# ethz-asl/laser_slam

Hardware: NVIDIA H100
Metric: ICP registrations/s (131072-pt scan vs 524288-pt map, 30 iterations) (higher is better)
Workload: dtype f32

## Files before the change

laser_slam_b200/csrc/ls_grid.cuh:

```cuda
#pragma once
#include <cfloat>
#include <climits>
#include <cstring>

#include <vector_types.h>
#include <vector_functions.h>

#include "ls_math.cuh"

#define LS_FB 8
#define LS_FB3 (LS_FB * LS_FB * LS_FB)
#define LS_PYR_LEVELS 7

namespace ls {

struct Entry {
  uint32_t start;
  int32_t meta;
};

struct Grid {
  float org[3];
  float H0, H1;
  float inv0, inv1;
// ... 113 lines not shown
}
LS_HD float cell_lo(float o, int c, float H) { return o + (float)c * H; }

LS_HD float gap(float q, float lo, float hi, float m) {
  const float a = (lo - m) - q;
  const float b = q - (hi + m);
  return fmaxf(0.0f, fmaxf(a, b));
}

#define LS_SHRINK 0.999999f

LS_HD float ball_radius(float best_d2, float margin) { return sqrtf(best_d2) * 1.000001f + margin; }

LS_HD void Best::offer_pt(float d, const float4& c, int p) { offer(d, f2i(c.w), p); }
LS_HD void TopK::offer_pt(float dist, const float4& c, int p) { offer(dist, f2i(c.w), p); }
template <class Acc>
LS_HD void consider_pt(const float4 p, int pos, float qx, float qy, float qz, Acc& b) {
  b.offer_pt(dist2(qx, qy, qz, p.x, p.y, p.z), p, pos);
}
template <class Acc>
LS_HD void consider(const float4* pts, int pos, float qx, float qy, float qz, Acc& b) {
  consider_pt(ld_pt(pts + pos), pos, qx, qy, qz, b);
}

template <class Acc>
LS_HD void scan_range(const float4* pts, uint32_t a, uint32_t e, float qx, float qy, float qz, Acc& b) {
  uint32_t pos = a;
  for (; pos + 4 <= e; pos += 4) {
    LS_CNT_STEP();
    const float4 p0 = ld_pt(pts + pos), p1 = ld_pt(pts + pos + 1), p2 = ld_pt(pts + pos + 2), p3 = ld_pt(pts + pos + 3);
    consider_pt(p0, (int)pos, qx, qy, qz, b);
    consider_pt(p1, (int)pos + 1, qx, qy, qz, b);
    consider_pt(p2, (int)pos + 2, qx, qy, qz, b);
    consider_pt(p3, (int)pos + 3, qx, qy, qz, b);
  }
  if (pos < e) LS_CNT_STEP();
  for (; pos < e; ++pos) consider(pts, (int)pos, qx, qy, qz, b);
}

template <class Acc>
LS_HD void visit_fine(const Grid& g, const Entry* tab, unsigned long long rows, float lox, float loy, float loz,
                      const float4* pts, float qx, float qy, float qz, Acc& b) {
  const float R = ball_radius(b.bound(), g.margin);
  const int x0 = coord_sub(qx - R, lox, g.inv1), x1 = coord_sub(qx + R, lox, g.inv1);
  const int y0 = coord_sub(qy - R, loy, g.inv1), y1 = coord_sub(qy + R, loy, g.inv1);
  const int z0 = coord_sub(qz - R, loz, g.inv1), z1 = coord_sub(qz + R, loz, g.inv1);
  for (int z = z0; z <= z1; ++z) {
    const float gz = gap(qz, cell_lo(loz, z, g.H1), cell_lo(loz, z + 1, g.H1), g.margin);
    const float gz2 = gz * gz;
    if (gz2 * LS_SHRINK > b.bound()) continue;
    const Entry* row = tab + (z * LS_FB + y0) * LS_FB;
    for (int y = y0; y <= y1; ++y, row += LS_FB) {
      if (!((rows >> (z * LS_FB + y)) & 1ull)) continue;
      const float gy = gap(qy, cell_lo(loy, y, g.H1), cell_lo(loy, y + 1, g.H1), g.margin);
      const float lb = gy * gy + gz2;
      if (lb * LS_SHRINK > b.bound()) continue;
      LS_CNT_STEP();
      const Entry e0 = ld_entry(row + x0);
      const Entry e1 = ld_entry(row + x1);
      scan_range(pts, e0.start, e1.start + (uint32_t)e1.meta, qx, qy, qz, b);
    }
  }
}

template <class Acc>
LS_HD void visit_top_entry(const Grid& g, const GridView& v, const Entry e, unsigned long long rows, float cx, float cy,
                           float cz, float qx, float qy, float qz, Acc& b) {
  if (e.meta > 0) {
    scan_range(v.pts, e.start, e.start + (uint32_t)e.meta, qx, qy, qz, b);
  } else if (e.meta < 0) {
    visit_fine(g, v.tab1 + (size_t)(~e.meta) * LS_FB3, rows, cx, cy, cz, v.pts, qx, qy, qz, b);
  }
}
template <class Acc>
LS_HD void visit_top_cell(const Grid& g, const GridView& v, int x, int y, int z, float cx, float cy, float cz, float qx,
                          float qy, float qz, Acc& b) {
  LS_CNT_STEP();
  const size_t ci = ((size_t)z * g.dim[1] + y) * g.dim[0] + x;
  const Entry e = ld_entry(v.top + ci);
  const unsigned long long rows = ld_rows(v.topmask + ci);
  visit_top_entry(g, v, e, rows, cx, cy, cz, qx, qy, qz, b);
}

template <class Acc>
LS_HDN void pyramid_query(const Grid& g, const GridView& v, float qx, float qy, float qz, Acc& b) {
  int lvl[LS_PYR_LEVELS + 1], bx[LS_PYR_LEVELS + 1], by[LS_PYR_LEVELS + 1], bz[LS_PYR_LEVELS + 1];
  unsigned long long mk[LS_PYR_LEVELS + 1];
  const int* td = g.pdim[g.n_pyr];
  const int n_top = td[0] * td[1] * td[2];
  for (int t = 0; t < n_top; ++t) {
    int sp = 0;
    lvl[0] = g.n_pyr;
    bx[0] = (t % td[0]) * 4;
    by[0] = ((t / td[0]) % td[1]) * 4;
    bz[0] = (t / (td[0] * td[1])) * 4;
    mk[0] = ld_mask(v.pyr + g.poff[g.n_pyr] + t);
    while (sp >= 0) {
      if (mk[sp] == 0ull) { --sp; continue; }
      const int bit = ctz64(mk[sp]);
      mk[sp] &= mk[sp] - 1ull;
      LS_CNT_STEP();
      const int cl = lvl[sp] - 1;
      const int cx = bx[sp] + (bit & 3), cy = by[sp] + ((bit >> 2) & 3), cz = bz[sp] + (bit >> 4);
      const float Hc = g.H0 * (float)(1 << (2 * cl));
      const float lx = cell_lo(g.org[0], cx, Hc), ly = cell_lo(g.org[1], cy, Hc), lz = cell_lo(g.org[2], cz, Hc);
      const float gx = gap(qx, lx, cell_lo(g.org[0], cx + 1, Hc), g.margin);
      const float gy = gap(qy, ly, cell_lo(g.org[1], cy + 1, Hc), g.margin);
      const float gz = gap(qz, lz, cell_lo(g.org[2], cz + 1, Hc), g.margin);
      const float lb = gx * gx + (gy * gy + gz * gz);
      if (lb * LS_SHRINK > b.bound()) continue;
      if (cl == 0) {
        visit_top_cell(g, v, cx, cy, cz, lx, ly, lz, qx, qy, qz, b);
      } else {
        ++sp;
        lvl[sp] = cl;
        bx[sp] = cx * 4; by[sp] = cy * 4; bz[sp] = cz * 4;
        mk[sp] = ld_mask(v.pyr + g.poff[cl] + ((size_t)cz * g.pdim[cl][1] + cy) * g.pdim[cl][0] + cx);
      }
    }
  }
}

template <class Acc>
LS_HD void ball_query(const Grid& g, const GridView& v, float qx, float qy, float qz, Acc& b) {
  const float R = ball_radius(b.bound(), g.margin);
  const int x0 = coord_top(qx - R, g.org[0], g.inv0, g.dim[0]), x1 = coord_top(qx + R, g.org[0], g.inv0, g.dim[0]);
  const int y0 = coord_top(qy - R, g.org[1], g.inv0, g.dim[1]), y1 = coord_top(qy + R, g.org[1], g.inv0, g.dim[1]);
  const int z0 = coord_top(qz - R, g.org[2], g.inv0, g.dim[2]), z1 = coord_top(qz + R, g.org[2], g.inv0, g.dim[2]);
  if ((x1 - x0 + 1) * (y1 - y0 + 1) * (z1 - z0 + 1) > 27 && g.n_pyr > 0) {
    pyramid_query(g, v, qx, qy, qz, b);
    return;
  }
  for (int z = z0; z <= z1; ++z) {
    const float cz = cell_lo(g.org[2], z, g.H0);
    const float gz = gap(qz, cz, cell_lo(g.org[2], z + 1, g.H0), g.margin);
    const float gz2 = gz * gz;
    if (gz2 * LS_SHRINK > b.bound()) continue;
    for (int y = y0; y <= y1; ++y) {
      const float cy = cell_lo(g.org[1], y, g.H0);
      const float gy = gap(qy, cy, cell_lo(g.org[1], y + 1, g.H0), g.margin);
      const float lbyz = gy * gy + gz2;
      if (lbyz * LS_SHRINK > b.bound()) continue;
      for (int x = x0; x <= x1; ++x) {
        const float cx = cell_lo(g.org[0], x, g.H0);
        const float gx = gap(qx, cx, cell_lo(g.org[0], x + 1, g.H0), g.margin);
        const float lb = gx * gx + lbyz;
        if (lb * LS_SHRINK > b.bound()) continue;
        visit_top_cell(g, v, x, y, z, cx, cy, cz, qx, qy, qz, b);
      }
    }
  }
}

LS_HDN void seed_query(const Grid& g, const GridView& v, float qx, float qy, float qz, Best& b) {
  const int cx = coord_top(qx, g.org[0], g.inv0, g.dim[0]);
  const int cy = coord_top(qy, g.org[1], g.inv0, g.dim[1]);
  const int cz = coord_top(qz, g.org[2], g.inv0, g.dim[2]);
  const Entry e = ld_entry(v.top + ((size_t)cz * g.dim[1] + cy) * g.dim[0] + cx);
  if (e.meta == 0) {
    int X = 0, Y = 0, Z = 0;
    const int* td = g.pdim[g.n_pyr];
    const int n_top = td[0] * td[1] * td[2];
    if (n_top > 1) {
      const float Ht = g.H0 * (float)(1 << (2 * g.n_pyr));
      float best_lb = INFINITY;
      for (int t = 0; t < n_top; ++t) {
        if (ld_mask(v.pyr + g.poff[g.n_pyr] + t) == 0ull) continue;
        const int tx = t % td[0], ty = (t / td[0]) % td[1], tz = t / (td[0] * td[1]);
        const float gx = gap(qx, cell_lo(g.org[0], tx, Ht), cell_lo(g.org[0], tx + 1, Ht), 0.f);
        const float gy = gap(qy, cell_lo(g.org[1], ty, Ht), cell_lo(g.org[1], ty + 1, Ht), 0.f);
        const float gz = gap(qz, cell_lo(g.org[2], tz, Ht), cell_lo(g.org[2], tz + 1, Ht), 0.f);
        const float lb = gx * gx + (gy * gy + gz * gz);
        if (lb < best_lb) { best_lb = lb; X = tx; Y = ty; Z = tz; }
      }
    }
    for (int l = g.n_pyr; l >= 1; --l) {
      unsigned long long mask = ld_mask(v.pyr + g.poff[l] + ((size_t)Z * g.pdim[l][1] + Y) * g.pdim[l][0] + X);
      const float Hc = g.H0 * (float)(1 << (2 * (l - 1)));
      float best_lb = INFINITY;
      int best_bit = -1;
      while (mask) {
        const int bit = ctz64(mask);
        mask &= mask - 1ull;
        const int ccx = X * 4 + (bit & 3), ccy = Y * 4 + ((bit >> 2) & 3), ccz = Z * 4 + (bit >> 4);
        const float gx = gap(qx, cell_lo(g.org[0], ccx, Hc), cell_lo(g.org[0], ccx + 1, Hc), 0.f);
        const float gy = gap(qy, cell_lo(g.org[1], ccy, Hc), cell_lo(g.org[1], ccy + 1, Hc), 0.f);
        const float gz = gap(qz, cell_lo(g.org[2], ccz, Hc), cell_lo(g.org[2], ccz + 1, Hc), 0.f);
        const float lb = gx * gx + (gy * gy + gz * gz);
        if (lb < best_lb) { best_lb = lb; best_bit = bit; }
      }
      if (best_bit < 0) return;
      X = X * 4 + (best_bit & 3);
      Y = Y * 4 + ((best_bit >> 2) & 3);
      Z = Z * 4 + (best_bit >> 4);
    }
    const Entry s0 = ld_entry(v.top + ((size_t)Z * g.dim[1] + Y) * g.dim[0] + X);
    if (s0.meta != 0) consider(v.pts, (int)s0.start, qx, qy, qz, b);
    return;
  }
  if (e.meta > 0) { scan_range(v.pts, e.start, e.start + (uint32_t)e.meta, qx, qy, qz, b); return; }
  const float lox = cell_lo(g.org[0], cx, g.H0), loy = cell_lo(g.org[1], cy, g.H0), loz = cell_lo(g.org[2], cz, g.H0);
  const int fx = coord_sub(qx, lox, g.inv1), fy = coord_sub(qy, loy, g.inv1), fz = coord_sub(qz, loz, g.inv1);
  const Entry* tab = v.tab1 + (size_t)(~e.meta) * LS_FB3;
  const Entry e1 = ld_entry(tab + (fz * LS_FB + fy) * LS_FB + fx);
  if (e1.meta != 0) { scan_range(v.pts, e1.start, e1.start + (uint32_t)e1.meta, qx, qy, qz, b); return; }
  const int xa = fx > 0 ? fx - 1 : 0, xb = fx < LS_FB - 1 ? fx + 1 : LS_FB - 1;
  for (int z = (fz > 0 ? fz - 1 : 0); z <= (fz < LS_FB - 1 ? fz + 1 : LS_FB - 1); ++z)
    for (int y = (fy > 0 ? fy - 1 : 0); y <= (fy < LS_FB - 1 ? fy + 1 : LS_FB - 1); ++y) {
      const Entry r0 = ld_entry(tab + (z * LS_FB + y) * LS_FB + xa);
      const Entry r1 = ld_entry(tab + (z * LS_FB + y) * LS_FB + xb);
      scan_range(v.pts, r0.start, r1.start + (uint32_t)r1.meta, qx, qy, qz, b);
    }
  if (b.pos < 0) consider(v.pts, (int)e.start, qx, qy, qz, b);
}

LS_HD Best nn_search(const Grid& g, const GridView& v, float qx, float qy, float qz, int warm_pos, float cap_d2) {
  Best b;
  b.d2 = cap_d2;
  b.idx = INT_MAX;
  b.pos = -1;
  if (g.m <= 0) { b.idx = -1; b.d2 = INFINITY; return b; }
  if (warm_pos >= 0) consider(v.pts, warm_pos, qx, qy, qz, b);
  else seed_query(g, v, qx, qy, qz, b);
  ball_query(g, v, qx, qy, qz, b);
  if (b.pos < 0) { b.idx = -1; b.d2 = INFINITY; }
  return b;
}

#ifndef LS_VK
#define LS_VK 8
#endif
static_assert(LS_VK <= 15, "the list header keeps the candidate count in 4 bits");
#ifndef LS_VL_ABS
#define LS_VL_ABS 0.0f
#endif
#ifndef LS_VL_REL
#define LS_VL_REL 0.5f
#endif
#ifndef LS_VL_SKIN
#define LS_VL_SKIN 4.0f
#endif
#ifndef LS_VL_GATE
#define LS_VL_GATE 1.0f
#endif
struct VLists {
  float4* vq;
  float4* vpts;
  int n;
};

struct Collector {
  float r2;
  int cnt;
  float4* out;
  int stride;
  LS_HD float bound() const { return r2; }
  LS_HD void offer_pt(float d, const float4& c, int p) {
    if (d <= r2) {
      if (cnt < LS_VK) st_state4(out + (size_t)cnt * stride, make_float4(c.x, c.y, c.z, i2f(p)));
      else r2 = -1.0f;
      ++cnt;
    }
  }
};

LS_HD bool vlist_query(const VLists& L, const float4* pts, int i, const float4 v, const float4 c0, float qx, float qy,
                       float qz, float cap_d2, Best& b, float4& cbest) {
  const unsigned int bits = (unsigned int)f2i(v.w);
  if (bits == 0u) return false;
  const int cnt = (int)(bits & 15u);
  const float Rv = i2f((int)(bits & ~15u));
  const float Rc = Rv * 0.999996f - sqrtf(dist2(qx, qy, qz, v.x, v.y, v.z)) * 1.000004f;
  if (!(Rc > 0.0f)) return false;
  b.d2 = cap_d2;
  b.idx = INT_MAX;
  b.pos = -1;
  auto take = [&](const float4 c) {
    const float d = dist2(qx, qy, qz, c.x, c.y, c.z);
    const int cpos = f2i(c.w);
    if (d < b.d2) {
      b.d2 = d;
      b.pos = cpos;
      cbest = c;
    } else if (d == b.d2) {
      if (b.pos < 0 || f2i(ld_pt(pts + cpos).w) < f2i(ld_pt(pts + b.pos).w)) {
        b.pos = cpos;
        cbest = c;
      }
    }
  };
  if (cnt > 0) take(c0);
  for (int k0 = 1; k0 < cnt; k0 += 4) {
    float4 cs[4];
#pragma unroll
    for (int u = 0; u < 4; ++u)
      cs[u] = k0 + u < cnt ? ld_state4(L.vpts + (size_t)(k0 + u) * L.n + i) : make_float4(0.f, 0.f, 0.f, 0.f);
#pragma unroll
    for (int u = 0; u < 4; ++u)
      if (k0 + u < cnt) take(cs[u]);
  }
  return b.d2 * 1.00001f <= Rc * Rc;
}

LS_HD void vlist_build(const Grid& g, const GridView& v, const VLists& L, int i, float qx, float qy, float qz, bool found,
                       float found_d2, float cap_d2, float motion) {
  float Rv;
  if (found) {
    const float want = sqrtf(found_d2);
    const float margin = fmaxf(want * LS_VL_REL, LS_VL_ABS) + 1e-4f;
    if (!(motion * LS_VL_GATE <= margin)) return;
    Rv = want + fminf(margin, fmaxf(0.002f, LS_VL_SKIN * motion));
  } else {
    const float want = sqrtf(cap_d2);
    if (!(motion <= want * 0.125f)) return;
    Rv = want * 1.05f + fminf(want * 0.25f, fmaxf(0.002f, 4.0f * motion));
  }
  if (!(Rv < 3.0e38f)) return;
  Collector c;
  c.r2 = Rv * Rv;
  c.cnt = 0;
  c.out = L.vpts + i;
  c.stride = L.n;
  ball_query(g, v, qx, qy, qz, c);
  float4 head = make_float4(qx, qy, qz, 0.0f);
  if (c.cnt <= LS_VK) head.w = i2f((int)((((unsigned int)f2i(Rv * 0.9999999f)) & ~15u) | (unsigned int)c.cnt));
  st_state4(L.vq + i, head);
}

LS_HDN void knn_search(const Grid& g, const GridView& v, float qx, float qy, float qz, int k, TopK& t) {
  t.reset(k);
  if (g.m <= 0) return;
  const float extent = g.H0 * (float)(g.dim[0] + g.dim[1] + g.dim[2]) + 1.0f;
  float R = g.H1;
  for (int round = 0; round < 64; ++round) {
    t.cap = R * R;
    ball_query(g, v, qx, qy, qz, t);
    if (t.d[k - 1] <= t.cap) break;
    if (R > extent + fabsf(qx - g.org[0]) + fabsf(qy - g.org[1]) + fabsf(qz - g.org[2])) break;
    R = R * 2.0f;
  }
}

LS_HD int top_index(const Grid& g, float x, float y, float z) {
  const int cx = coord_top(x, g.org[0], g.inv0, g.dim[0]);
  const int cy = coord_top(y, g.org[1], g.inv0, g.dim[1]);
  const int cz = coord_top(z, g.org[2], g.inv0, g.dim[2]);
  return (cz * g.dim[1] + cy) * g.dim[0] + cx;
}
LS_HD void top_origin(const Grid& g, int c0, float& lox, float& loy, float& loz) {
  const int cx = c0 % g.dim[0];
  const int cy = (c0 / g.dim[0]) % g.dim[1];
  const int cz = c0 / (g.dim[0] * g.dim[1]);
  lox = cell_lo(g.org[0], cx, g.H0);
  loy = cell_lo(g.org[1], cy, g.H0);
  loz = cell_lo(g.org[2], cz, g.H0);
}
LS_HD int sub_index(float x, float y, float z, float lox, float loy, float loz, float inv) {
  return (coord_sub(z, loz, inv) * LS_FB + coord_sub(y, loy, inv)) * LS_FB + coord_sub(x, lox, inv);
}

LS_HDN void grid_setup(Grid& g, const float* lo, const float* hi, float cell_size, int max_cells, int leaf_split,
                       int m) {
  float H = cell_size > 0.f ? cell_size : 2.0f;
  float ext[3], emax = 0.f, oabs = 0.f;
  for (int a = 0; a < 3; ++a) {
    ext[a] = hi[a] - lo[a];
    if (!(ext[a] >= 0.f)) ext[a] = 0.f;
    emax = fmaxf(emax, ext[a]);
    oabs = fmaxf(oabs, fmaxf(fabsf(lo[a]), fabsf(hi[a])));
  }
  for (int it = 0; it < 40; ++it) {
    const float inv = 1.0f / H;
    double cells = 1.0;
    for (int a = 0; a < 3; ++a) cells *= (double)floorf(ext[a] * inv) + 1.0;
    if (cells <= (double)max_cells) break;
    H = H * 2.0f;
  }
  g.H0 = H;
  g.H1 = H / (float)LS_FB;
  g.inv0 = 1.0f / g.H0;
  g.inv1 = 1.0f / g.H1;
  int n = 1;
  for (int a = 0; a < 3; ++a) {
    g.org[a] = lo[a];
    int d = (int)floorf(ext[a] * g.inv0) + 1;
    if (d < 1) d = 1;
    g.dim[a] = d;
    n *= d;
  }
  g.n_cells0 = n;
  g.margin = (oabs + emax + H) * 1.9073486328125e-06f;
  g.m = m;
  g.leaf_split = leaf_split > 0 ? leaf_split : 32;
  g.n_tab1 = 0;
  g.overflow = 0;
  for (int a = 0; a < 3; ++a) g.pdim[0][a] = g.dim[a];
  g.poff[0] = 0;
  int off = 0, l = 0;
  do {
    ++l;
    for (int a = 0; a < 3; ++a) g.pdim[l][a] = (g.pdim[l - 1][a] + 3) / 4;
    g.poff[l] = off;
    off += g.pdim[l][0] * g.pdim[l][1] * g.pdim[l][2];
  } while ((g.pdim[l][0] > 1 || g.pdim[l][1] > 1 || g.pdim[l][2] > 1) && l < LS_PYR_LEVELS);
  g.n_pyr = l;
  g.n_pyr_cells = off;
}

}
```

laser_slam_b200/csrc/ls_kernels.cuh:

```cuda
#pragma once
#include <cuda_runtime.h>
#include <cooperative_groups.h>

#include "ls_grid.cuh"

namespace ls {

constexpr int kMaxParts = 16;
constexpr int kScanTile = 4096;
constexpr int kScanThreads = 512;
constexpr int kIcpThreads = 512;
constexpr int kIcpCtasPerSm = 1024 / kIcpThreads;
constexpr int kMaxSmooth = 15;
constexpr uint32_t kTag1 = 1u << 31, kKeyMask = (1u << 31) - 1u;
constexpr int kSubShift = 22;
constexpr uint32_t kCellMask = (1u << kSubShift) - 1u;

struct Parts {
  int n_parts;
  int offset[kMaxParts + 1];
  const float4* pts[kMaxParts];
  const float4* nrm[kMaxParts];
  float T[kMaxParts][16];
  int identity[kMaxParts];
// ... 772 lines not shown
__global__ void __launch_bounds__(128) knn_normals_kernel(const BuildState* __restrict__ bs, GridView view,
                                                           const float4* __restrict__ pts ,
                                                           int n, int k, float4* __restrict__ out) {
  __shared__ Grid g;
  if (threadIdx.x == 0) g = bs->grid;
  __syncthreads();
  auto centred = [&](int j) {
    float4 p = __ldg(pts + j);
    p.x = p.x - g.mu[0];
    p.y = p.y - g.mu[1];
    p.z = p.z - g.mu[2];
    return p;
  };
  for (int i = blockIdx.x * blockDim.x + threadIdx.x; i < n; i += gridDim.x * blockDim.x) {
    const float4 q = centred(i);
    TopK t;
    knn_search(g, view, q.x, q.y, q.z, k, t);
    int cnt = 0;
    double mx = 0.0, my = 0.0, mz = 0.0;
    for (int j = 0; j < k; ++j) {
      if (t.id[j] == INT_MAX) break;
      const float4 p = centred(t.id[j]);
      mx = mx + (double)p.x;
      my = my + (double)p.y;
      mz = mz + (double)p.z;
      ++cnt;
    }
    float4 nn = make_float4(0.f, 0.f, 0.f, 0.f);
    if (cnt >= 3) {
      const double inv = 1.0 / (double)cnt;
      mx = mx * inv; my = my * inv; mz = mz * inv;
      double C[9] = {0, 0, 0, 0, 0, 0, 0, 0, 0};
      for (int j = 0; j < cnt; ++j) {
        const float4 p = centred(t.id[j]);
        const double dx = (double)p.x - mx, dy = (double)p.y - my, dz = (double)p.z - mz;
        C[0] = C[0] + dx * dx; C[1] = C[1] + dx * dy; C[2] = C[2] + dx * dz;
        C[4] = C[4] + dy * dy; C[5] = C[5] + dy * dz; C[8] = C[8] + dz * dz;
      }
      C[3] = C[1]; C[6] = C[2]; C[7] = C[5];
      double nv[3];
      smallest_eigvec3(C, nv);
      const double ox = (double)q.x + (double)g.mu[0], oy = (double)q.y + (double)g.mu[1], oz = (double)q.z + (double)g.mu[2];
      const double dot = nv[0] * ox + (nv[1] * oy + nv[2] * oz);
      const double sgn = dot > 0.0 ? -1.0 : 1.0;
      nn = make_float4((float)(sgn * nv[0]), (float)(sgn * nv[1]), (float)(sgn * nv[2]), 0.f);
    }
    out[i] = nn;
  }
}

__device__ __forceinline__ unsigned long long globaltimer_ns() {
  unsigned long long t;
  asm volatile("mov.u64 %0, %%globaltimer;" : "=l"(t));
  return t;
}
#define LS_STAMP(slot)                                                                   \
  do {                                                                                   \
    if (P.phase_ns && cta == 0 && tid == 0) P.phase_ns[iter * 6 + (slot)] = globaltimer_ns(); \
  } while (0)

__device__ __forceinline__ unsigned int ld_relaxed_u32(const unsigned int* p) {
  unsigned int v;
  asm volatile("ld.relaxed.gpu.global.u32 %0, [%1];" : "=r"(v) : "l"(p) : "memory");
  return v;
}
__device__ __forceinline__ void red_release_inc(unsigned int* p) {
  asm volatile("red.release.gpu.global.add.u32 [%0], 1;" ::"l"(p) : "memory");
}
__device__ __forceinline__ unsigned int ld_relaxed_sys_u32(const unsigned int* p) {
  unsigned int v;
  asm volatile("ld.relaxed.sys.global.u32 %0, [%1];" : "=r"(v) : "l"(p) : "memory");
  return v;
}
__device__ __forceinline__ unsigned long long ld_relaxed_sys_u64(const unsigned long long* p) {
  unsigned long long v;
  asm volatile("ld.relaxed.sys.global.u64 %0, [%1];" : "=l"(v) : "l"(p) : "memory");
  return v;
}
__device__ __forceinline__ void red_release_sys_inc(unsigned int* p) {
  asm volatile("red.release.sys.global.add.u32 [%0], 1;" ::"l"(p) : "memory");
}

__device__ __forceinline__ void problem_barrier(unsigned int* ctr, unsigned int n_ctas, unsigned int& epoch) {
  __syncthreads();
  if (threadIdx.x == 0) {
    epoch += n_ctas;
    red_release_inc(ctr);
    unsigned int polls = 0;
    unsigned long long t0 = 0ull;
    while (ld_relaxed_u32(ctr) < epoch) {
      __nanosleep(64);
      if ((++polls & 0x3fffu) == 0u) {
        const unsigned long long now = globaltimer_ns();
        if (t0 == 0ull) t0 = now;
        else if (now - t0 > 8000000000ull) {
          printf("[ls] icp_kernel barrier timeout: block %d waits for %u, counter %u\n", (int)blockIdx.x, epoch, ld_relaxed_u32(ctr));
          __trap();
        }
      }
    }
  }
  __syncthreads();
}

struct SelectOut {
  unsigned int bin, rem, total;
};
constexpr size_t kWorkWords = sizeof(IcpWork) / 4;
static_assert(sizeof(IcpWork) % 16 == 0 && offsetof(IcpWork, hist) % 16 == 0 && offsetof(IcpWork, acc) % 16 == 0, "sections move as uint4");

__device__ __forceinline__ void shard_exchange(const IcpProblem& P, IcpWork* X, int cta, unsigned int G, unsigned int& epoch,
                                               unsigned int& xepoch, int off0, int n0, int off1, int n1, int off2, int n2) {
  problem_barrier(&X->barrier, G, epoch);
  const int peers = P.shard_count - 1;
  if (cta < peers) {
    const int g = cta + (cta >= P.shard_rank ? 1 : 0);
    const uint4* src = reinterpret_cast<const uint4*>(X);
    uint4* dst = reinterpret_cast<uint4*>(P.link.peer_slots[g] + P.shard_rank);
    for (int k = threadIdx.x; k < n0 / 4; k += kIcpThreads) __stcg(dst + off0 / 4 + k, __ldcg(src + off0 / 4 + k));
    for (int k = threadIdx.x; k < n1 / 4; k += kIcpThreads) __stcg(dst + off1 / 4 + k, __ldcg(src + off1 / 4 + k));
    for (int k = threadIdx.x; k < n2 / 4; k += kIcpThreads) __stcg(dst + off2 / 4 + k, __ldcg(src + off2 / 4 + k));
    __syncthreads();
    if (threadIdx.x == 0) {
      __threadfence_system();
      red_release_sys_inc(P.link.peer_flag[g]);
    }
  }
  xepoch += (unsigned int)peers;
  if (threadIdx.x == 0) {
    const unsigned int target = P.link.flag_base + xepoch;
    unsigned int polls = 0;
    unsigned long long t0 = 0ull;
    while ((int)(ld_relaxed_sys_u32(P.link.flag) - target) < 0) {
      __nanosleep(64);
      if ((++polls & 0x3fffu) == 0u) {
        const unsigned long long now = globaltimer_ns();
        if (t0 == 0ull) t0 = now;
        else if (now - t0 > 8000000000ull) {
          printf("[ls] icp_kernel shard %d: a peer did not arrive (block %d waits for %u, counter %u)\n", P.shard_rank, (int)blockIdx.x,
                 target, ld_relaxed_sys_u32(P.link.flag));
          __trap();
        }
      }
    }
  }
  __syncthreads();
}

__device__ __forceinline__ unsigned long long sum_slots_u64(const unsigned long long* p, int n_slots) {
  unsigned long long v = 0ull;
  for (int g = 0; g < n_slots; ++g) v += __ldcg(p + (size_t)g * (kWorkWords / 2));
  return v;
}

__device__ __forceinline__ void block_select(const unsigned int* ghist, int nbins, unsigned int k, bool first,
                                             float ratio, SelectOut* out, unsigned int* ws, int n_slots = 1) {
  const int per = nbins / kIcpThreads;
  unsigned int c[2048 / kIcpThreads], loc = 0;
  for (int j = 0; j < per; ++j) {
    unsigned int v = 0;
    for (int g = 0; g < n_slots; ++g) v += __ldcg(ghist + (size_t)g * kWorkWords + threadIdx.x * per + j);
    c[j] = v;
    loc += v;
  }
  unsigned int incl = loc;
  const int lane = threadIdx.x & 31, warp = threadIdx.x >> 5;
  for (int o = 1; o < 32; o <<= 1) {
    const unsigned int v = __shfl_up_sync(0xffffffffu, incl, o);
    if (lane >= o) incl += v;
  }
  __syncthreads();
  if (lane == 31) ws[warp] = incl;
  __syncthreads();
  unsigned int woff = 0, total = 0;
  for (int w = 0; w < kIcpThreads / 32; ++w) {
    const unsigned int v = ws[w];
    if (w < warp) woff += v;
    total += v;
  }
  if (first) {
    k = (unsigned int)((float)total * ratio);
    if (total > 0 && k >= total) k = total - 1;
  }
  unsigned int run = woff + incl - loc;
  for (int j = 0; j < per; ++j) {
    if (k >= run && k < run + c[j]) {
      out->bin = threadIdx.x * per + j;
      out->rem = k - run;
    }
    run += c[j];
  }
  if (threadIdx.x == 0) out->total = total;
  __syncthreads();
}


struct SelHists {
  unsigned int h1[1024];
  unsigned int h2[2048];
  unsigned int h3[1024];
};
constexpr unsigned int kNoPrediction = 0xffffffffu;

__device__ __forceinline__ void phase_a_record(const IcpProblem& P, int i, const Best& b, SelHists* H, unsigned int pred_bin1,
                                               unsigned int pred_pref12) {
  if (b.pos >= 0) __stcg(P.pos + i, b.pos);
  const float d = b.pos >= 0 ? b.d2 : INFINITY;
  __stcg(P.d2 + i, d);
  const unsigned int key = __float_as_uint(d);
  if (key <= 0x7f800000u) {
    atomicAdd(&H->h1[key >> 21], 1u);
    if ((key >> 21) == pred_bin1) {
      atomicAdd(&H->h2[(key >> 10) & 2047u], 1u);
      if ((key >> 10) == pred_pref12) atomicAdd(&H->h3[key & 1023u], 1u);
    }
  }
}

__device__ __forceinline__ void residual_terms(float sx, float sy, float sz, const float4 q, const float4 nn, float* f, float& e) {
  float u = sy * nn.z, v = sz * nn.y;
  f[0] = u - v;
  u = sz * nn.x; v = sx * nn.z;
  f[1] = u - v;
  u = sx * nn.y; v = sy * nn.x;
  f[2] = u - v;
  f[3] = nn.x; f[4] = nn.y; f[5] = nn.z;
  const float dx = sx - q.x, dy = sy - q.y, dz = sz - q.z;
  e = dx * nn.x;
  float t = dy * nn.y;
  e = e + t;
  t = dz * nn.z;
  e = e + t;
}

constexpr int kPairSlots = 64;
constexpr int kIcpPairBytes = (kIcpThreads / 32) * kPairSlots * 8 * (int)sizeof(float);
__constant__ unsigned char kPairRow[32] = {0, 0, 0, 0, 0, 0, 1, 1, 1, 1, 1, 2, 2, 2, 2, 3, 3, 3, 4, 4, 5, 0, 1, 2, 3, 4, 5, 7, 7, 7, 7, 7};
__constant__ unsigned char kPairCol[32] = {0, 1, 2, 3, 4, 5, 1, 2, 3, 4, 5, 2, 3, 4, 5, 3, 4, 5, 4, 5, 5, 6, 6, 6, 6, 6, 6, 7, 7, 7, 7, 7};

struct PairQueue {
  float* recs;
  int head, cnt;
  long long acc;
};

__device__ __noinline__ long long consume_pairs(const float* recs, int head, int count, long long acc) {
  const int lane = threadIdx.x & 31;
  const int ro = kPairRow[lane], co = kPairCol[lane];
  const float scale = lane < 27 ? 4194304.0f : 1.0f;
#pragma unroll 4
  for (int j = 0; j < count; ++j) {
    const float* r = recs + ((head + j) & (kPairSlots - 1)) * 8;
    const float a = r[ro], b = r[co], sg = r[7];
    long long v = __float2ll_rn((a * b) * scale);
    if (sg < 0.f) v = -v;
    acc += v;
  }
  return acc;
}

__device__ __forceinline__ void push_pairs(const IcpProblem& P, PairQueue& Q, int sign, float sx, float sy, float sz,
                                           const float4 q, int pos) {
  const unsigned int m = __ballot_sync(0xffffffffu, sign != 0);
  if (m == 0u) return;
  if (sign) {
    float f[6], e;
    residual_terms(sx, sy, sz, q, __ldg(P.nrm + pos), f, e);
    const int slot = (Q.head + Q.cnt + __popc(m & ((1u << (threadIdx.x & 31)) - 1u))) & (kPairSlots - 1);
    float4* r = reinterpret_cast<float4*>(Q.recs + slot * 8);
    r[0] = make_float4(f[0], f[1], f[2], f[3]);
    r[1] = make_float4(f[4], f[5], e, (float)sign);
  }
  Q.cnt += __popc(m);
  __syncwarp();
  if (Q.cnt >= 32) {
    Q.acc = consume_pairs(Q.recs, Q.head, 32, Q.acc);
    Q.head = (Q.head + 32) & (kPairSlots - 1);
    Q.cnt -= 32;
    __syncwarp();
  }
}

__device__ __forceinline__ void drain_pairs(PairQueue& Q, unsigned long long* slab) {
  if (Q.cnt > 0) {
    Q.acc = consume_pairs(Q.recs, Q.head, Q.cnt, Q.acc);
    Q.head = (Q.head + Q.cnt) & (kPairSlots - 1);
    Q.cnt = 0;
  }
  const int lane = threadIdx.x & 31;
  if (lane < 28) slab[lane] = (unsigned long long)Q.acc;
  Q.acc = 0ll;
  __syncwarp();
}

__device__ __noinline__ void phase_a_search(const Grid* gp, const IcpProblem* Pp, const float* T_iter, const float* T_prev,
                                            int i, float cap, SelHists* H, unsigned int pred_bin1, unsigned int pred_pref12) {
  if (i < 0) return;
  const Grid& g = *gp;
  const IcpProblem& P = *Pp;
  const float4 r = __ldg(P.rd + i);
  float sx, sy, sz;
  xform_point(T_iter, r.x, r.y, r.z, sx, sy, sz);
  const int warm = __ldcg(P.pos + i);
  const Best b = nn_search(g, P.view, sx, sy, sz, warm, cap);
  phase_a_record(P, i, b, H, pred_bin1, pred_pref12);
  if (T_prev) {
    float px, py, pz;
    xform_point(T_prev, r.x, r.y, r.z, px, py, pz);
    vlist_build(g, P.view, P.lists, i, sx, sy, sz, b.pos >= 0, b.d2, cap, sqrtf(dist2(sx, sy, sz, px, py, pz)));
  }
}

__device__ __forceinline__ void push_searched(const IcpProblem& P, PairQueue& Q, const float* T_iter, int j, float acc_limit) {
  if (!(acc_limit >= 0.0f)) return;
  float d = INFINITY;
  if (j >= 0) d = __ldcg(P.d2 + j);
  const bool keep = d <= acc_limit;
  if (__ballot_sync(0xffffffffu, keep) == 0u) return;
  float4 q = make_float4(0.f, 0.f, 0.f, 0.f);
  float sx = 0.f, sy = 0.f, sz = 0.f;
  int pos = -1;
  if (keep) {
    pos = __ldcg(P.pos + j);
    const float4 r = __ldg(P.rd + j);
    xform_point(T_iter, r.x, r.y, r.z, sx, sy, sz);
    q = __ldg(P.view.pts + pos);
  }
  push_pairs(P, Q, keep ? 1 : 0, sx, sy, sz, q, pos);
}

__device__ __noinline__ void final_match(const Grid* gp, const IcpProblem* Pp, const float* T, int i) {
  if (i < 0) return;
  const IcpProblem& P = *Pp;
  const float4 r = __ldg(P.rd + i);
  float sx, sy, sz;
  xform_point(T, r.x, r.y, r.z, sx, sy, sz);
  const Best b = nn_search(*gp, P.view, sx, sy, sz, __ldcg(P.pos + i), INFINITY);
  const uint32_t orig = __ldg(P.qperm + i);
  P.d2_out[orig] = b.d2;
  P.ids[orig] = b.idx;
}

__device__ __forceinline__ void flush_slabs(unsigned long long (*acc_w)[28], unsigned long long* gacc) {
  __syncthreads();
  if (threadIdx.x < 28) {
    unsigned long long t = 0ull;
#pragma unroll
    for (int w = 0; w < kIcpThreads / 32; ++w) t += acc_w[w][threadIdx.x];
    if (t != 0ull) atomicAdd(&gacc[threadIdx.x], t);
  }
  __syncthreads();
}

__device__ __forceinline__ void flush_hist(const unsigned int* hs, int nbins, unsigned int* gh) {
  for (int k = threadIdx.x; k < nbins; k += kIcpThreads) {
    const unsigned int v = hs[k];
    if (v) atomicAdd(&gh[k], v);
  }
}

__global__ void __launch_bounds__(kIcpThreads, kIcpCtasPerSm)
icp_kernel(const IcpProblem* __restrict__ probs, int ctas_per_problem, IcpParamsDev prm, int dynamic) {
  const int pi = blockIdx.x / ctas_per_problem;
  const int cta = blockIdx.x - pi * ctas_per_problem;
  const IcpProblem& P = probs[pi];
  IcpWork* W = P.work;
  const bool xg = P.shard_count > 1;
  IcpWork* X = xg ? P.link.slots + P.shard_rank : W;
  const IcpWork* S0 = xg ? P.link.slots : W;
  const int n_slots = xg ? P.shard_count : 1;
  const unsigned int G = (unsigned int)ctas_per_problem;
  unsigned int xepoch = 0;
  const int tid = threadIdx.x, lane = tid & 31;

  __shared__ Grid g;
  __shared__ float T_iter[16], T_last[16];
  __shared__ SelHists hs;
  __shared__ unsigned long long acc_w[kIcpThreads / 32][28];
  __shared__ SelectOut sel;
  __shared__ unsigned int ws[kIcpThreads / 32];
  __shared__ double qh[kMaxSmooth + 2][4];
  __shared__ double th[kMaxSmooth + 2][3];
  __shared__ int flag_stop, flag_status;
  __shared__ int miss_buf[kIcpThreads / 32][64];
  extern __shared__ __align__(16) float pair_buf[];

  if (tid == 0) {
    g = P.bs->grid;
    for (int i = 0; i < 16; ++i) T_iter[i] = (i % 5 == 0) ? 1.f : 0.f;
    quat_from_T(T_iter, qh[0]);
    th[0][0] = th[0][1] = th[0][2] = 0.0;
    flag_stop = 0;
    flag_status = 0;
  }
  __syncthreads();
  PairQueue Q;
  Q.recs = pair_buf + (tid >> 5) * (kPairSlots * 8);
  Q.head = 0;
  Q.cnt = 0;
  Q.acc = 0ll;

  const int n = P.n;
  int chunk = (n + (int)G - 1) / (int)G;
  chunk = (chunk + 31) & ~31;
  const int q_begin = min(n, cta * chunk), q_end = min(n, q_begin + chunk);

  for (int i = q_begin + tid; i < q_end; i += kIcpThreads) {
    __stcg(P.pos + i, -1);
    __stcg(P.lists.vq + i, make_float4(0.f, 0.f, 0.f, 0.f));
  }

  float cap = 0.04f;
  int redo = 0;
  unsigned int epoch = 0;
  constexpr int kHistOff = (int)(offsetof(IcpWork, hist) / 4), kAccOff = (int)(offsetof(IcpWork, acc) / 4);
  auto meet = [&](int off0, int n0, int off1, int n1, int off2, int n2) {
    if (xg) shard_exchange(P, X, cta, G, epoch, xepoch, off0, n0, off1, n1, off2, n2);
    else problem_barrier(&X->barrier, G, epoch);
  };
  problem_barrier(&X->barrier, G, epoch);
  int hist_count = 1;
  int iter = 0, converged = 0, max_reached = 0, last_kept = 0;
  float last_limit = 0.f;
  unsigned int pred_bin1 = kNoPrediction, pred_pref12 = kNoPrediction;
  float acc_limit = -1.0f;

  for (;;) {
    const int par = iter & 1;
    LS_STAMP(0);
    for (int k = tid; k < (int)(sizeof(SelHists) / 4); k += kIcpThreads) reinterpret_cast<unsigned int*>(&hs)[k] = 0u;
    __syncthreads();
    {
      const float* T_prev = iter >= 1 ? T_last : nullptr;
      int* mq = miss_buf[tid >> 5];
      int n_miss = 0;
      int next = q_begin + (tid & ~31);
      for (;;) {
        int base;
        if (dynamic) {
          unsigned int bb = 0;
          if (lane == 0) bb = atomicAdd(&W->qctr[par], 32u);
          bb = __shfl_sync(0xffffffffu, bb, 0);
          if (bb >= (unsigned int)n) break;
          base = (int)bb;
        } else {
          if (next >= q_end) break;
          base = next;
          next += kIcpThreads;
        }
        const int i = base + lane;
        bool valid = i < (dynamic ? n : q_end);
        if (redo && valid) valid = !(__ldcg(P.d2 + i) < INFINITY);
        bool hit = false;
        Best b;
        b.d2 = INFINITY; b.idx = INT_MAX; b.pos = -1;
        float4 c = make_float4(0.f, 0.f, 0.f, 0.f);
        float sx = 0.f, sy = 0.f, sz = 0.f;
        if (valid) {
          const float4 r = __ldg(P.rd + i);
          const float4 v = __ldcg(P.lists.vq + i);
          const float4 c0 = __ldcg(P.lists.vpts + i);
          xform_point(T_iter, r.x, r.y, r.z, sx, sy, sz);
          hit = vlist_query(P.lists, P.view.pts, i, v, c0, sx, sy, sz, cap, b, c);
          if (hit) phase_a_record(P, i, b, &hs, pred_bin1, pred_pref12);
        }
        push_pairs(P, Q, (hit && b.pos >= 0 && b.d2 <= acc_limit) ? 1 : 0, sx, sy, sz, c, b.pos);
        const unsigned int mm = __ballot_sync(0xffffffffu, valid && !hit);
        if (mm) {
          if (valid && !hit) mq[n_miss + __popc(mm & ((1u << lane) - 1u))] = i;
          n_miss += __popc(mm);
          __syncwarp();
          if (n_miss >= 32) {
            n_miss -= 32;
            const int j = mq[n_miss + lane];
            __syncwarp();
            phase_a_search(&g, &P, T_iter, T_prev, j, cap, &hs, pred_bin1, pred_pref12);
            push_searched(P, Q, T_iter, j, acc_limit);
          }
        }
      }
      if (n_miss > 0) {
        __syncwarp();
        const int j = lane < n_miss ? mq[lane] : -1;
        phase_a_search(&g, &P, T_iter, T_prev, j, cap, &hs, pred_bin1, pred_pref12);
        __syncwarp();
        push_searched(P, Q, T_iter, j, acc_limit);
      }
    }
    drain_pairs(Q, acc_w[tid >> 5]);
    flush_slabs(acc_w, X->acc[par]);
    flush_hist(hs.h1, 1024, X->hist[par][0]);
    if (pred_bin1 != kNoPrediction) {
      flush_hist(hs.h2, 2048, X->hist[par][3]);
      flush_hist(hs.h3, 1024, X->hist[par][4]);
    }
    {
      const int hb = kHistOff + par * 5 * 2048;
      const bool pr = pred_bin1 != kNoPrediction;
      meet(hb, 1024, hb + 3 * 2048, pr ? 2048 : 0, hb + 4 * 2048, pr ? 1024 : 0);
    }
    LS_STAMP(1);

    block_select(S0->hist[par][0], 1024, 0u, true, prm.trim_ratio, &sel, ws, n_slots);
    if (sel.total == 0u) {
      if (tid == 0) { flag_status = 1; if (cta == 0) W->fail_code = 1; }
      __syncthreads();
      break;
    }
    if (sel.bin >= 1020u) {
      if (!(cap < INFINITY)) {
        if (tid == 0) { flag_status = 1; if (cta == 0) W->fail_code = 1; }
        __syncthreads();
        break;
      }
      cap = cap < 64.0f ? cap * 4.0f : INFINITY;
      ++redo;
      meet(0, 0, 0, 0, 0, 0);
      if (cta == 0 && tid == 0) {
        X->hist[par][0][1020] = 0u;
        W->qctr[par] = 0u;
      }
      problem_barrier(&X->barrier, G, epoch);
      continue;
    }
    const unsigned int bin1 = sel.bin, rem1 = sel.rem;
    if (cta == 0) {
      unsigned int* h = &X->hist[par ^ 1][0][0];
      for (int k = tid; k < 5 * 2048; k += kIcpThreads) h[k] = 0u;
      if (tid < 32) X->acc[par ^ 1][tid] = 0ull;
    }
    if (cta == 0 && tid == 0) W->qctr[par ^ 1] = 0u;
    const bool spec2 = bin1 == pred_bin1;
    if (!spec2) {
      for (int k = tid; k < 2048; k += kIcpThreads) hs.h2[k] = 0u;
      __syncthreads();
      for (int i = q_begin + tid; i < q_end; i += kIcpThreads) {
        const unsigned int key = __float_as_uint(__ldcg(P.d2 + i));
        if (key < 0x7f800000u && (key >> 21) == bin1) atomicAdd(&hs.h2[(key >> 10) & 2047u], 1u);
      }
      __syncthreads();
      flush_hist(hs.h2, 2048, X->hist[par][1]);
      meet(kHistOff + (par * 5 + 1) * 2048, 2048, 0, 0, 0, 0);
    }
    LS_STAMP(2);
    block_select(S0->hist[par][spec2 ? 3 : 1], 2048, rem1, false, 0.f, &sel, ws, n_slots);
    const unsigned int bin2 = sel.bin, rem2 = sel.rem;
    const unsigned int prefix12 = (bin1 << 11) | bin2;
    const bool spec3 = spec2 && prefix12 == pred_pref12;
    if (!spec3) {
      for (int k = tid; k < 1024; k += kIcpThreads) hs.h3[k] = 0u;
      __syncthreads();
      for (int i = q_begin + tid; i < q_end; i += kIcpThreads) {
        const unsigned int key = __float_as_uint(__ldcg(P.d2 + i));
        if (key < 0x7f800000u && (key >> 10) == prefix12) atomicAdd(&hs.h3[key & 1023u], 1u);
      }
      __syncthreads();
      flush_hist(hs.h3, 1024, X->hist[par][2]);
      meet(kHistOff + (par * 5 + 2) * 2048, 1024, 0, 0, 0, 0);
    }
    LS_STAMP(3);
    block_select(S0->hist[par][spec3 ? 4 : 2], 1024, rem2, false, 0.f, &sel, ws, n_slots);
    const float limit = __uint_as_float((prefix12 << 10) | sel.bin);
    cap = fmaxf(limit * (iter == 0 ? 0.5f : 2.0f), 1e-12f);
    redo = 0;

    for (int base = q_begin; base < q_end; base += kIcpThreads) {
      const int i = base + tid;
      int sign = 0, pos = -1;
      if (i < q_end) {
        const float d = __ldcg(P.d2 + i);
        pos = __ldcg(P.pos + i);
        sign = ((d <= limit && pos >= 0) ? 1 : 0) - ((d <= acc_limit) ? 1 : 0);
      }
      if (__ballot_sync(0xffffffffu, sign != 0) == 0u) continue;
      float sx = 0.f, sy = 0.f, sz = 0.f;
      float4 q = make_float4(0.f, 0.f, 0.f, 0.f);
      if (sign) {
        const float4 r = __ldg(P.rd + i);
        xform_point(T_iter, r.x, r.y, r.z, sx, sy, sz);
        q = __ldg(P.view.pts + pos);
      }
      push_pairs(P, Q, sign, sx, sy, sz, q, pos);
    }
    drain_pairs(Q, acc_w[tid >> 5]);
    flush_slabs(acc_w, X->acc[par]);
    meet(kAccOff + par * 64, 64, 0, 0, 0, 0);
    LS_STAMP(4);

    if (tid == 0) {
      double A[36], b[6], x[6];
      int k = 0;
      for (int rr = 0; rr < 6; ++rr)
        for (int cc = rr; cc < 6; ++cc, ++k) {
          const double v = (double)(long long)sum_slots_u64(&S0->acc[par][k], n_slots) / 4194304.0;
          A[rr * 6 + cc] = v;
          A[cc * 6 + rr] = v;
        }
      for (int rr = 0; rr < 6; ++rr) b[rr] = -((double)(long long)sum_slots_u64(&S0->acc[par][21 + rr], n_slots) / 4194304.0);
      last_kept = (int)sum_slots_u64(&S0->acc[par][27], n_slots);
      last_limit = limit;
      int status = 0, stop = 0;
      if (last_kept == 0) {
        status = 1;
        if (cta == 0) W->fail_code = 2;
      } else {
        if (!chol6(A, b, x)) jacobi_pinv_solve6(A, b, x);
        for (int i = 0; i < 6; ++i)
          if (!is_finite_d(x[i])) status = 1;
        if (status && cta == 0) W->fail_code = 3;
      }
      if (cta == 0) {
        W->dbg_total = sel.total; W->dbg_bin[0] = bin1; W->dbg_bin[1] = bin2; W->dbg_bin[2] = sel.bin;
        W->dbg_rem[0] = rem1; W->dbg_rem[1] = rem2; W->dbg_rem[2] = sel.rem;
// ... 76 lines not shown
```

Baseline: 981.1.

## Fuse nearest-neighbor search with Verlet list collection into one ball query

Instead of running a nearest-neighbor search and then a separate ball query to build the per-point Verlet candidate list, a combined collector feeds both the best-match tracker and the list collector in a single grid traversal. The list radius is now computed from the warm-start or seed estimate rather than the final nearest distance, so it may be larger or smaller than before. This saves one grid traversal per point in iterations that rebuild lists. The trade-off is that the combined search bound is the max of the best distance and the list radius, so the NN search cannot shrink its cutoff as aggressively, and list contents may differ.

```diff
diff --git a/laser_slam_b200/csrc/ls_grid.cuh b/laser_slam_b200/csrc/ls_grid.cuh
--- a/laser_slam_b200/csrc/ls_grid.cuh
+++ b/laser_slam_b200/csrc/ls_grid.cuh
@@ -439,29 +439,69 @@
   return b.d2 * 1.00001f <= Rc * Rc;
 }
 
-LS_HD void vlist_build(const Grid& g, const GridView& v, const VLists& L, int i, float qx, float qy, float qz, bool found,
-                       float found_d2, float cap_d2, float motion) {
+LS_HD float vlist_radius(bool found, float found_d2, float cap_d2, float motion) {
   float Rv;
   if (found) {
     const float want = sqrtf(found_d2);
     const float margin = fmaxf(want * LS_VL_REL, LS_VL_ABS) + 1e-4f;
-    if (!(motion * LS_VL_GATE <= margin)) return;
+    if (!(motion * LS_VL_GATE <= margin)) return 0.0f;
     Rv = want + fminf(margin, fmaxf(0.002f, LS_VL_SKIN * motion));
   } else {
     const float want = sqrtf(cap_d2);
-    if (!(motion <= want * 0.125f)) return;
+    if (!(motion <= want * 0.125f)) return 0.0f;
     Rv = want * 1.05f + fminf(want * 0.25f, fmaxf(0.002f, 4.0f * motion));
   }
-  if (!(Rv < 3.0e38f)) return;
+  return Rv < 3.0e38f ? Rv : 0.0f;
+}
+
+LS_HD void vlist_head(const VLists& L, int i, float qx, float qy, float qz, float Rv, int cnt) {
+  float4 head = make_float4(qx, qy, qz, 0.0f);
+  if (cnt <= LS_VK) head.w = i2f((int)((((unsigned int)f2i(Rv * 0.9999999f)) & ~15u) | (unsigned int)cnt));
+  st_state4(L.vq + i, head);
+}
+
+LS_HD void vlist_build(const Grid& g, const GridView& v, const VLists& L, int i, float qx, float qy, float qz, bool found,
+                       float found_d2, float cap_d2, float motion) {
+  const float Rv = vlist_radius(found, found_d2, cap_d2, motion);
+  if (!(Rv > 0.0f)) return;
   Collector c;
   c.r2 = Rv * Rv;
   c.cnt = 0;
   c.out = L.vpts + i;
   c.stride = L.n;
   ball_query(g, v, qx, qy, qz, c);
-  float4 head = make_float4(qx, qy, qz, 0.0f);
-  if (c.cnt <= LS_VK) head.w = i2f((int)((((unsigned int)f2i(Rv * 0.9999999f)) & ~15u) | (unsigned int)c.cnt));
-  st_state4(L.vq + i, head);
+  vlist_head(L, i, qx, qy, qz, Rv, c.cnt);
+}
+
+struct SearchCollect {
+  Best best;
+  Collector list;
+  LS_HD float bound() const { return fmaxf(best.d2, list.r2); }
+  LS_HD void offer_pt(float d, const float4& c, int p) {
+    best.offer_pt(d, c, p);
+    list.offer_pt(d, c, p);
+  }
+};
+
+LS_HD Best nn_search_collect(const Grid& g, const GridView& v, const VLists& L, int i, float qx, float qy, float qz,
+                             int warm_pos, float cap_d2, float motion) {
+  SearchCollect s;
+  Best& b = s.best;
+  b.d2 = cap_d2;
+  b.idx = INT_MAX;
+  b.pos = -1;
+  if (g.m <= 0) { b.idx = -1; b.d2 = INFINITY; return b; }
+  if (warm_pos >= 0) consider(v.pts, warm_pos, qx, qy, qz, b);
+  else seed_query(g, v, qx, qy, qz, b);
+  const float Rv = vlist_radius(b.pos >= 0, b.d2, cap_d2, motion);
+  s.list.r2 = Rv > 0.0f ? Rv * Rv : -1.0f;
+  s.list.cnt = 0;
+  s.list.out = L.vpts + i;
+  s.list.stride = L.n;
+  ball_query(g, v, qx, qy, qz, s);
+  if (Rv > 0.0f) vlist_head(L, i, qx, qy, qz, Rv, s.list.cnt);
+  if (b.pos < 0) { b.idx = -1; b.d2 = INFINITY; }
+  return b;
 }
 
 LS_HDN void knn_search(const Grid& g, const GridView& v, float qx, float qy, float qz, int k, TopK& t) {
diff --git a/laser_slam_b200/csrc/ls_kernels.cuh b/laser_slam_b200/csrc/ls_kernels.cuh
--- a/laser_slam_b200/csrc/ls_kernels.cuh
+++ b/laser_slam_b200/csrc/ls_kernels.cuh
@@ -1098,13 +1098,15 @@
   float sx, sy, sz;
   xform_point(T_iter, r.x, r.y, r.z, sx, sy, sz);
   const int warm = __ldcg(P.pos + i);
-  const Best b = nn_search(g, P.view, sx, sy, sz, warm, cap);
-  phase_a_record(P, i, b, H, pred_bin1, pred_pref12);
+  Best b;
   if (T_prev) {
     float px, py, pz;
     xform_point(T_prev, r.x, r.y, r.z, px, py, pz);
-    vlist_build(g, P.view, P.lists, i, sx, sy, sz, b.pos >= 0, b.d2, cap, sqrtf(dist2(sx, sy, sz, px, py, pz)));
-  }
+    b = nn_search_collect(g, P.view, P.lists, i, sx, sy, sz, warm, cap, sqrtf(dist2(sx, sy, sz, px, py, pz)));
+  } else {
+    b = nn_search(g, P.view, sx, sy, sz, warm, cap);
+  }
+  phase_a_record(P, i, b, H, pred_bin1, pred_pref12);
 }
 
 __device__ __forceinline__ void push_searched(const IcpProblem& P, PairQueue& Q, const float* T_iter, int j, float acc_limit) {
```

Result: faster. 1048, median of 6 (+6.8%).
